# DeJhon-Huang/TrueTrace-Unity-Pathtracer

Measured on AMD Instinct MI355X. Metric: Mrays/sec (primary+1-bounce) on Sponza CWBVH at 1080p; % HBM roofline, higher is better.
Workload: dtype f32

## Files before the change

### truetrace-unity-pathtracer_amd/csrc/tt_trace.hip

```cpp
#include "tt_launch.h"
#include "tt_wide.h"

#ifndef TT_LEAF_REFILL_MIN
#define TT_LEAF_REFILL_MIN (TT_LEAF_POOL ? 16 : TT_REFILL_MIN)
#endif

namespace {
template <int INFO, int LEAF = 0>
__device__ __forceinline__ bool write_record(const TraceArgs& A, uint32_t ray_index, uint32_t pix, float col_w,
                                             const Best& best, const LaneRay& wr, int32_t inst_mesh = 0,
                                             int32_t inst_tri_offset = 0) {
    tt_ray_data* R = A.rays + ray_index;
    const int32_t best_mesh = LEAF ? (best.tri_id != -1 ? inst_mesh : 0) : best.mesh_id;
    auto tri_offset_of_best = [&]() -> int32_t {
        if (LEAF) return best.tri_id != -1 ? inst_tri_offset : A.mesh[0].TriOffset;
        return A.mesh[best.mesh_id].TriOffset;
    };
    if (INFO != 0) {
        if (pix < A.n_pixels) {
            uint4 o;
            bool write = false;
            if (INFO == 1) {
                const int32_t to = tri_offset_of_best();
                o = make_uint4((uint32_t)best_mesh, (uint32_t)(best.tri_id - to),
// ... 28 lines not shown
                        } else {
                            o.x = __float_as_uint(w.dx * best.t + w.ox);
                            o.y = __float_as_uint(w.dy * best.t + w.oy);
                            o.z = __float_as_uint(w.dz * best.t + w.oz);
                        }
                    }
                    o.w = miss ? 1u : 0u;
                }
            }
            if (write) reinterpret_cast<uint4*>(A.info)[pix] = o;
        }
    }
    const uint32_t uv = (uint32_t)(best.u * 65535.0f) | ((uint32_t)(best.v * 65535.0f) << 16);
    const uint4 hit = make_uint4((uint32_t)best_mesh, (uint32_t)best.tri_id, __float_as_uint(best.t), uv);
    reinterpret_cast<uint4*>(R)[2] = hit;
    if (A.hits_out) {
        const u32x4 v = {hit.x, hit.y, hit.z, hit.w};
        __builtin_amdgcn_raw_buffer_store_b128(v, buffer_rsrc(A.hits_out, 0x7fffffff), (ray_index - A.ray_offset) << 4,
                                               0, 0);
    }
    return best.t != A.far_plane;
}

__device__ __forceinline__ void keep_record(const TraceArgs& A, uint32_t ray_index) {
    if (A.hits_out) {
        const uint4 h = reinterpret_cast<const uint4*>(A.rays + ray_index)[2];
        const u32x4 v = {h.x, h.y, h.z, h.w};
        __builtin_amdgcn_raw_buffer_store_b128(v, buffer_rsrc(A.hits_out, 0x7fffffff), (ray_index - A.ray_offset) << 4,
                                               0, 0);
    }
}

static_assert(TT_CHUNK_BIG == 64, "the adaptive order maps one dequeue (TT_CHUNK_BIG rays) to one 64-ray chunk");
#ifndef TT_ORDER_MIN_REPS
#define TT_ORDER_MIN_REPS 32
#endif
__device__ __forceinline__ void record_chunk_cost(const TraceArgs& A, bool swizzle, uint32_t ray_index, int32_t reps) {
    if (reps < TT_ORDER_MIN_REPS) return;
    const uint32_t local = ray_index - A.ray_offset;
    uint32_t c = local >> 6;
    if (swizzle) {
        const uint32_t py = fastdiv(local, A.div_width), px = local - py * A.width;
        c = (py >> 3) * (A.width >> 3) + (px >> 3);
    }
    atomicMax(A.chunk_cost + c, (uint32_t)reps);
}
}


namespace {
__device__ __forceinline__ bool root_leaf_hit(const RootLeaf& R, const LaneRay& r, float max_distance) {
    const float adjx = __uint_as_float(rl_byte(R.e, 0) << 23) * r.ix;
    const float adjy = __uint_as_float(rl_byte(R.e, 1) << 23) * r.iy;
    const float adjz = __uint_as_float(rl_byte(R.e, 2) << 23) * r.iz;
    const float orgx = r.ix * (R.px - r.ox);
    const float orgy = r.iy * (R.py - r.oy);
    const float orgz = r.iz * (R.pz - r.oz);
    const bool nx = r.dx < 0.0f, ny = r.dy < 0.0f, nz = r.dz < 0.0f;
    const uint32_t x_min = rl_byte(nx ? R.qhi : R.qlo, 0), x_max = rl_byte(nx ? R.qlo : R.qhi, 0);
    const uint32_t y_min = rl_byte(ny ? R.qhi : R.qlo, 1), y_max = rl_byte(ny ? R.qlo : R.qhi, 1);
    const uint32_t z_min = rl_byte(nz ? R.qhi : R.qlo, 2), z_max = rl_byte(nz ? R.qlo : R.qhi, 2);
    const float tminx = fma_((float)x_min, adjx, orgx);
    const float tminy = fma_((float)y_min, adjy, orgy);
    const float tminz = fma_((float)z_min, adjz, orgz);
    const float tmaxx = fma_((float)x_max, adjx, orgx);
    const float tmaxy = fma_((float)y_max, adjy, orgy);
    const float tmaxz = fma_((float)z_max, adjz, orgz);
    const float tmin = fmaxf(fmaxf(tminx, tminy), fmaxf(tminz, 1e-8f));
    float tmaxz_c;
    asm("v_min_f32 %0, %1, %2" : "=v"(tmaxz_c) : "v"(tmaxz), "v"(max_distance));
    const float tmax = fminf(fminf(tmaxx, tmaxy), tmaxz_c);
    return tmin < tmax;
}
}


template <bool STATS, bool MATCHECK, int INFO, bool IND, bool ORD, int LEAF = 0>
__device__ __forceinline__ void trace_body(const TraceArgs& A) {
    static_assert(!LEAF || (!STATS && !MATCHECK && !ORD), "the leaf-TLAS form has no stats / material / order variants");
    constexpr bool POOL = LEAF != 0 && TT_LEAF_POOL != 0;
    constexpr bool ROOTSTEP = POOL && TT_LEAF_ROOT_STEP != 0;
    constexpr bool RESTART = ROOTSTEP && TT_LEAF_RESTART != 0;
    static_assert(!RESTART || LEAF == 1, "the restart parks no world ray: the record write reads it back");
    constexpr int tt_lds_depth = lds_depth_of<LEAF>();
    static_assert(!POOL || TT_CHUNK_BIG == TT_WAVE, "the prepared-ray pool holds one chunk, one slot per lane");
    __shared__ uint2 s_stack[tt_lds_depth][TT_BLOCK];
    __shared__ uint4 s_pool[POOL ? 3 : 1][TT_BLOCK];
    (void)s_pool;
    LeafEntry L{};
    if (LEAF) L = load_leaf_mesh<true>(A.leaf, A.root.base_tri + firstbithigh(A.root.bits));
    uint32_t root_cg_x = 0, root_tg_x = 0, root_imask = 0;
    if (ROOTSTEP) {
        const NodeWords n = load_node_uniform(A.nodes, A.n_nodes, (uint32_t)L.off.w);
        root_cg_x = n.n1.x + (uint32_t)L.off.y;
        root_tg_x = n.n1.y + (uint32_t)L.off.x;
        root_imask = n.n0.w >> 24;
    }
    const uint32_t tid = threadIdx.x;
    zero_next_control(A.ctl_next, tid);
    const uint32_t gtid = blockIdx.x * TT_BLOCK + tid;
    const uint32_t spill_stride = gridDim.x * TT_BLOCK;
    uint2* __restrict__ spill = A.spill;
    (void)gtid;
    (void)spill_stride;
    (void)spill;
    const uint32_t lane = tid & (TT_WAVE - 1);
#ifdef TT_DIAG_BLOCKS
    if (tid < TT_DB_N) tt_db[tid] = 0ull;
    __syncthreads();
#endif

    uint32_t pool_next = 0, pool_end = 0, more = 1;
    const uint32_t wave_id = blockIdx.x * (TT_BLOCK / TT_WAVE) + (tid >> 6);
    SegState S{blockIdx.x % TT_SEGS, 0u, 0u};
    const uint32_t n_rays = IND ? launch_ray_count(A) : A.n_rays;
    const uint32_t n_tiles = (n_rays + 63u) >> 6;
    const bool swizzle = IND ? (A.tile_swizzle && n_rays == A.n_pixels) : (A.tile_swizzle != 0u);
    const __amdgpu_buffer_rsrc_t nodes = buffer_rsrc(A.nodes, A.n_nodes * (uint32_t)TT_NODE_STRIDE);
    const __amdgpu_buffer_rsrc_t tris = buffer_rsrc(A.tris, A.n_tris * (uint32_t)sizeof(TriPos));

    constexpr uint32_t TT_IDLE = 0x80000000u;
    uint32_t ray_index = 0;
    uint32_t pix = 0;
    float col_w = 0.0f;
    bool pending = false;
    LaneRay ray{}, wray{};
    Best best{};
    uint2 cg = make_uint2(0u, 0u), tg = make_uint2(0u, TT_IDLE);
    uint32_t oct = 0;
    int32_t stack_size = 0, tlas_ss = -1;
    int32_t NodeOffset = 0, TriOffset = 0, MatOffset = 0, mesh_id = -1, Reps = 0;
    if (LEAF) {
        NodeOffset = L.off.y;
        TriOffset = L.off.x;
        MatOffset = L.off.z;
        mesh_id = L.mesh_id;
    }
    uint32_t c_nodes = 0, c_tris = 0, c_blas = 0, c_acc = 0, c_rays = 0, c_hits = 0, c_reps = 0, c_ovf = 0;
    uint32_t d_iter = 0, d_node_lanes = 0, d_node_iters = 0, d_tri_lanes = 0, d_tri_iters = 0, d_active_lanes = 0;
    uint32_t d_lead_same = 0, d_uniform = 0;
    auto world_ray = [&]() -> LaneRay { return wray; };
    auto ray_of = [&](uint32_t widx) -> uint32_t {
        uint32_t local = widx;
        if (swizzle) {
            const uint32_t tw = A.width >> 3;
            const uint32_t t = widx >> 6, l = widx & 63u;
            const uint32_t ty = fastdiv(t, A.div_tiles), tx = t - ty * tw;
            local = (ty * 8u + (l >> 3)) * A.width + tx * 8u + (l & 7u);
        }
        return A.ray_offset + local;
    };
    (void)ray_of;
    uint64_t parked = 0ull;
    (void)parked;
    auto ray_index_of = [&](uint32_t v) -> uint32_t {
        if constexpr (RESTART) return ray_of(v);
        return v;
    };

#if TT_ROOT_LEAF
    const bool rl_ok = A.root.ok != 0u;
#endif
    auto enter_blas = [&]() {
            TT_DB(8);
            const uint32_t mo = firstbithigh(tg.y);
            tg.y &= ~(1u << mo);
            const LeafEntry e = load_leaf_mesh<true>(A.leaf, tg.x + mo);
            mesh_id = e.mesh_id;
            NodeOffset = e.off.y;
            TriOffset = e.off.x;
            bool ok = true;
            if (tg.y != 0u) TT_PUSH(tg, ok);
            if (ok && (cg.y & 0xff000000u)) TT_PUSH(cg, ok);
            tg.y = 0u;
            if (ok) {
                tlas_ss = stack_size;
                MatOffset = e.off.z;
                enter_object_space(e, ray, oct, cg);
                if (STATS) c_blas++;
            } else {
                tg.y = TT_IDLE;
                if (STATS) c_ovf++;
                TT_REPORT_OVERFLOW(A);
                keep_record(A, ray_index);
            }
    };
    auto finish_ray = [&]() {
        const bool hit = write_record<INFO, LEAF>(A, ray_index_of(ray_index), pix, col_w, best, world_ray(), mesh_id,
                                                  TriOffset);
        if (STATS) c_hits += hit ? 1u : 0u;
        (void)hit;
        if (ORD) record_chunk_cost(A, swizzle, ray_index, Reps);
    };
    auto start_from = [&](const uint32_t widx, const uint4 p0, const uint4 p1, const uint4 p2) {
        TT_DL(19, true);
        ray_index = RESTART ? widx : ray_of(widx);
        ray.ox = __uint_as_float(p0.x);
        ray.oy = __uint_as_float(p0.y);
        ray.oz = __uint_as_float(p0.z);
        ray.dx = __uint_as_float(p0.w);
        ray.dy = __uint_as_float(p1.x);
        ray.dz = __uint_as_float(p1.y);
        ray.ix = __uint_as_float(p1.z);
        ray.iy = __uint_as_float(p1.w);
        ray.iz = __uint_as_float(p2.x);
        pix = p2.y;
        if (ROOTSTEP) {
            col_w = -1.0f;
            oct = p2.z & 0x7fffffffu;
            const uint32_t inner = p2.w & 0xff000000u;
            cg = make_uint2(root_cg_x, inner ? (inner | root_imask) : 0u);
            tg = make_uint2(root_tg_x, p2.w & 0x00ffffffu);
            Reps = (p2.z & 0x80000000u) ? 2 : 1;
        } else {
            col_w = __uint_as_float(p2.z);
            oct = p2.w & 0x7fffffffu;
            cg = make_uint2((p2.w & 0x80000000u) ? (uint32_t)L.off.w : 0u, p2.w & 0x80000000u);
        }
        if (LEAF == 2) {
            const uint4* rp = reinterpret_cast<const uint4*>(A.rays + ray_index);
            const uint4 r0 = rp[0], r1 = rp[1];
            wray.ox = __uint_as_float(r0.x);
            wray.oy = __uint_as_float(r0.y);
            wray.oz = __uint_as_float(r0.z);
            wray.dx = __uint_as_float(r1.x);
            wray.dy = __uint_as_float(r1.y);
            wray.dz = __uint_as_float(r1.z);
        }
        best.t = A.far_plane;
        best.u = 0.0f;
        best.v = 0.0f;
        best.mesh_id = 0;
        best.tri_id = -1;
        if (!ROOTSTEP) tg = make_uint2(0u, 0u);
        stack_size = 0;
        if (!ROOTSTEP) Reps = 1;
    };
    (void)start_from;
    constexpr uint32_t REFILL_MIN = LEAF ? TT_LEAF_REFILL_MIN : TT_REFILL_MIN;
    while (true) {
        TT_DB(0);
        const uint64_t idle = __ballot((int32_t)tg.y < 0);
        const uint32_t n_idle = (uint32_t)__builtin_popcount((uint32_t)idle) + (uint32_t)__builtin_popcount((uint32_t)(idle >> 32));
        const bool pool_dry = !more && pool_next >= pool_end;
#if TT_DRAIN_PRIO
        if (pool_dry) __builtin_amdgcn_s_setprio(TT_DRAIN_PRIO);
#endif
        const bool to_wide = TT_WIDE && pool_dry && n_idle < TT_WAVE && TT_WAVE - n_idle <= TT_WIDE_ENTER;
        const uint32_t refill_min = RESTART && pool_next >= pool_end ? (uint32_t)TT_LEAF_RESTART_MIN : REFILL_MIN;
        if ((n_idle == TT_WAVE && pool_dry) || (n_idle >= refill_min && !pool_dry) || to_wide) {
            if (pending) {
                TT_DB(1);
                finish_ray();
                pending = false;
            }
            if constexpr (RESTART) {
                if (parked != 0ull) {
                    TT_DB(34);
                    if ((parked >> lane) & 1ull) {
                        TT_DL(35, true);
                        const uint4 k0 = s_pool[0][tid];
                        const uint2 k1 = reinterpret_cast<const uint2*>(&s_pool[1][tid])[0];
                        Best kb;
                        kb.tri_id = (int32_t)k0.x;
                        kb.t = __uint_as_float(k0.y);
                        kb.u = __uint_as_float(k0.z);
                        kb.v = __uint_as_float(k0.w);
                        kb.mesh_id = 0;
                        write_record<INFO, LEAF>(A, ray_of(k1.x), k1.y, -1.0f, kb, LaneRay{}, mesh_id, TriOffset);
                    }
                    parked = 0ull;
                    __builtin_amdgcn_fence(__ATOMIC_ACQ_REL, "wavefront");
                    __builtin_amdgcn_wave_barrier();
                }
            }
        }
        if (n_idle == TT_WAVE && pool_dry) break;
#if TT_WIDE
        if (to_wide) {
            TT_DB(13);
            WideState st{{ray, world_ray(), cg, tg, oct, stack_size, tlas_ss, NodeOffset, TriOffset, MatOffset, Reps,
                          ray_index_of(ray_index), tid, gtid, (int32_t)tg.y >= 0},
                         best, mesh_id, pix, col_w};
            regroup<2, LEAF>(st, __ballot((int32_t)tg.y >= 0), lane);
            auto finish_wide = [&](const WideState& w) {
                const bool hit = write_record<INFO, LEAF>(A, w.ray_index, w.pix, w.col_w, w.best, w.wray, mesh_id, TriOffset);
                if (STATS) c_hits += hit ? 1u : 0u;
                if (ORD) record_chunk_cost(A, swizzle, w.ray_index, w.Reps);
            };
            auto exhaust_wide = [&](const WideState& w, bool overflow) {
                keep_record(A, w.ray_index);
                if (ORD && !overflow) record_chunk_cost(A, swizzle, w.ray_index, w.Reps);
            };
            wide_phase<STATS, MATCHECK, 2, LEAF>(A, st, s_stack, spill, spill_stride, nodes, tris, lane,
                                           Counters{c_nodes, c_tris, c_blas, c_acc, c_hits, c_reps, c_ovf},
                                           finish_wide, exhaust_wide);
            break;
        }
#endif
        if (n_idle >= refill_min && !pool_dry) {
            TT_DB(2);
#if TT_LONG_PRIO
            if (__ballot((int32_t)tg.y >= 0 && Reps >= TT_LONG_PRIO) != 0ull) __builtin_amdgcn_s_setprio(TT_LONG_PRIO_LEVEL);
            else __builtin_amdgcn_s_setprio(0);
#endif
            const uint32_t avail = pool_end - pool_next;
            uint32_t new_base = 0, new_count = 0;
            if (avail < n_idle && more) {
                new_count = sched_reserve(A.ctl, n_rays, n_tiles, lane, n_idle - avail, wave_id, S, new_base);
                more = new_count > 0 ? 1u : 0u;
                if (ORD && A.order && new_count > 0)
                    new_base = (__builtin_amdgcn_readfirstlane(A.order[new_base >> 6]) << 6) | (new_base & 63u);
            }
            const PoolTake pt = pool_take<TT_UNIFORM_POOL != 0>(idle, n_idle, new_base, new_count, pool_next, pool_end, more);
            const uint32_t widx = pt.widx;
            pool_next = pt.pool_next;
            pool_end = pt.pool_end;
            more = pt.more;
            if constexpr (POOL) {
                const uint32_t pcol = tid - lane;
                const bool take = (int32_t)tg.y < 0 && widx != 0xffffffffu;
                const bool take_left = take && lane_prefix(idle) < min(avail, n_idle);
                auto start_ray = [&](const uint4 p0, const uint4 p1, const uint4 p2) { start_from(widx, p0, p1, p2); };
                uint4 p0 = make_uint4(0u, 0u, 0u, 0u), p1 = p0, p2 = p0;
                if (take_left) {
                    const uint32_t slot = pcol + (widx & 63u);
                    p0 = s_pool[0][slot];
                    p1 = s_pool[1][slot];
                    p2 = s_pool[2][slot];
                    if (ROOTSTEP) start_ray(p0, p1, p2);
                }
                __builtin_amdgcn_fence(__ATOMIC_ACQ_REL, "wavefront");
                __builtin_amdgcn_wave_barrier();
                if (new_count > 0) {
                    TT_DB(4);
                    uint4 q0 = make_uint4(0u, 0u, 0u, 0u), q1 = q0, q2 = q0;
                    NodeWords rn{};
                    if (ROOTSTEP) rn = load_node_uniform(A.nodes, A.n_nodes, (uint32_t)L.off.w);
                    if (lane < new_count) {
                        const uint4* rp = reinterpret_cast<const uint4*>(A.rays + ray_of(new_base + lane));
                        const uint4 r0 = rp[0], r1 = rp[1];
                        float cw = 0.0f;
                        if (INFO == 2) cw = (r0.w < A.n_pixels) ? A.colors[r0.w].Data[3] : 0.0f;
                        LaneRay r;
                        r.ox = __uint_as_float(r0.x);
                        r.oy = __uint_as_float(r0.y);
                        r.oz = __uint_as_float(r0.z);
                        r.dx = __uint_as_float(r1.x);
                        r.dy = __uint_as_float(r1.y);
                        r.dz = __uint_as_float(r1.z);
                        r.ix = rcp_rn(r.dx);
                        r.iy = rcp_rn(r.dy);
                        r.iz = rcp_rn(r.dz);
                        uint32_t o = 0u;
                        uint2 g = make_uint2(0u, 0u);
                        const bool root_hit = root_leaf_hit(A.root, r, A.far_plane);
                        TT_DL(29, root_hit);
                        if (root_hit) enter_object_space(L, r, o, g);
                        q0 = make_uint4(__float_as_uint(r.ox), __float_as_uint(r.oy), __float_as_uint(r.oz),
                                        __float_as_uint(r.dx));
                        q1 = make_uint4(__float_as_uint(r.dy), __float_as_uint(r.dz), __float_as_uint(r.ix),
                                        __float_as_uint(r.iy));
                        q2 = make_uint4(__float_as_uint(r.iz), r0.w, __float_as_uint(cw), o | g.y);
                        if (ROOTSTEP) {
                            if (INFO == 2 && !(cw == -1.0f || (float)A.bounce == cw)) q2.y = 0xffffffffu;
                            q2.z = o | g.y;
                            q2.w = 0u;
                            s_pool[0][tid] = q0;
                            s_pool[1][tid] = q1;
                            s_pool[2][tid] = q2;
                            if (root_hit) {
                                TT_DB(28);
                                s_pool[2][tid].w = node_intersect(rn.n0, rn.n1, rn.n2, rn.n3, rn.n4, r, o, A.far_plane);
                            }
                        }
                    }
                    if (!ROOTSTEP) {
                        s_pool[0][tid] = q0;
                        s_pool[1][tid] = q1;
                        s_pool[2][tid] = q2;
                    }
                }
                __builtin_amdgcn_fence(__ATOMIC_ACQ_REL, "wavefront");
                __builtin_amdgcn_wave_barrier();
                if (take && !take_left) {
                    const uint32_t slot = pcol + (widx & 63u);
                    p0 = s_pool[0][slot];
                    p1 = s_pool[1][slot];
                    p2 = s_pool[2][slot];
                    if (ROOTSTEP) start_ray(p0, p1, p2);
                }
                if (!ROOTSTEP && take) start_ray(p0, p1, p2);
            }
            if (!POOL && (int32_t)tg.y < 0 && widx != 0xffffffffu) {
                TT_DB(4);
                TT_DL(19, true);
                uint32_t local = widx;
                if (swizzle) {
                    const uint32_t tw = A.width >> 3;
                    const uint32_t t = widx >> 6, l = widx & 63u;
                    const uint32_t ty = fastdiv(t, A.div_tiles), tx = t - ty * tw;
                    local = (ty * 8u + (l >> 3)) * A.width + tx * 8u + (l & 7u);
                }
                ray_index = A.ray_offset + local;
                const uint4* rp = reinterpret_cast<const uint4*>(A.rays + ray_index);
                const uint4 r0 = rp[0], r1 = rp[1];
                pix = r0.w;
                if (INFO == 2) col_w = (pix < A.n_pixels) ? A.colors[pix].Data[3] : 0.0f;
                ray.ox = __uint_as_float(r0.x);
                ray.oy = __uint_as_float(r0.y);
                ray.oz = __uint_as_float(r0.z);
                ray.dx = __uint_as_float(r1.x);
                ray.dy = __uint_as_float(r1.y);
                ray.dz = __uint_as_float(r1.z);
                ray.ix = rcp_rn(ray.dx);
                ray.iy = rcp_rn(ray.dy);
                ray.iz = rcp_rn(ray.dz);
                best.t = A.far_plane;
                best.u = 0.0f;
                best.v = 0.0f;
                best.mesh_id = 0;
                best.tri_id = -1;
                tg = make_uint2(0u, 0u);
                stack_size = 0;
                if (LEAF) {
                    if (LEAF == 2) wray = ray;
                    cg = make_uint2(0u, 0u);
                    Reps = 1;
                    if (root_leaf_hit(A.root, ray, best.t)) enter_object_space(L, ray, oct, cg);
                }
                if (!LEAF) {
                    wray = ray;
                    oct = octant_inv4(ray);
                    cg = make_uint2(A.tlas_base, 0x80000000u);
                    tlas_ss = -1;
                    NodeOffset = (int32_t)A.tlas_base;
                    TriOffset = 0;
                    MatOffset = 0;
                    mesh_id = -1;
                    Reps = 0;
                }
                if (STATS) c_rays++;
#if TT_ROOT_LEAF
                if (!LEAF && rl_ok) {
                    const RootLeaf& RL = A.root;
                    const bool hit = root_leaf_hit(RL, ray, best.t);
                    cg = make_uint2(RL.base_child, 0u);
                    tg = make_uint2(RL.base_tri, hit ? RL.bits : 0u);
                    Reps = 1;
                    if (STATS) c_nodes++;
                    if (hit) enter_blas();
                }
#endif
            }
        }

        TT_DL(30, (int32_t)tg.y < 0);
        if (STATS) {
            const uint64_t nm = __ballot(tg.y == 0u && Reps < TT_MAX_REPS && (cg.y & 0xff000000u));
            const uint64_t am = __ballot((int32_t)tg.y >= 0);
            if (lane == 0) {
                d_iter++;
                d_node_lanes += (uint32_t)__popcll(nm);
                d_node_iters += nm ? 1u : 0u;
                d_active_lanes += (uint32_t)__popcll(am);
            }
        }
        if (tg.y == 0u) {
            TT_DB(5);
            if (Reps >= TT_MAX_REPS) {
                tg.y = TT_IDLE;
                if (STATS) c_reps++;
                keep_record(A, ray_index_of(ray_index));
                if (ORD) record_chunk_cost(A, swizzle, ray_index, Reps);
            } else if (cg.y & 0xff000000u) {
                const uint32_t child = take_child(cg, oct);
                bool ok = true;
                if (cg.y & 0xff000000u) {
                    TT_DB(7);
                    TT_PUSH(cg, ok);
                }
                if (ok) {
                    TT_DB(6);
                    TT_DL(17, true);
                    if (STATS) {
                        const uint32_t lead = __builtin_amdgcn_readfirstlane(child);
                        const uint64_t same = __ballot(child == lead), all = __ballot(true);
                        d_lead_same += child == lead ? 1u : 0u;
                        d_uniform += (same == all && lane == (uint32_t)__builtin_ctzll(all)) ? 1u : 0u;
                    }
                    const NodeWords n = load_node<TT_NODE_CPOL>(nodes, child);
                    const uint32_t hitmask = node_intersect(n.n0, n.n1, n.n2, n.n3, n.n4, ray, oct, best.t);
                    cg = node_group(hitmask, n, NodeOffset);
                    tg = tri_group(hitmask, n, TriOffset);
                    Reps++;
                    if (STATS) c_nodes++;
                } else {
                    tg.y = TT_IDLE;
                    if (STATS) c_ovf++;
                    TT_REPORT_OVERFLOW(A);
                    keep_record(A, ray_index_of(ray_index));
                }
            } else {
                tg = cg;
                cg = make_uint2(0u, 0u);
            }
            if (!LEAF && (int32_t)tg.y > 0 && tlas_ss == -1) enter_blas();
        }

        if (STATS) {
            const uint64_t tm = __ballot((int32_t)tg.y > 0);
            if (lane == 0) {
                d_tri_lanes += (uint32_t)__popcll(tm);
                d_tri_iters += tm ? 1u : 0u;
            }
        }
        if ((int32_t)tg.y > 0) {
            TT_DB(9);
            TT_DL(18, true);
            const uint32_t ti = firstbithigh(tg.y);
            tg.y &= ~(1u << ti);
            const bool acc = intersect_triangle<MATCHECK>(tris, A.mat, A.bounce == 0, A.flags, (int32_t)(tg.x + ti),
                                                          mesh_id, MatOffset, ray, best);
            if (STATS) {
                c_tris++;
                c_acc += acc ? 1u : 0u;
            }
        }

        if constexpr (RESTART) {
            const bool used_up = tg.y == 0u && (cg.y & 0xff000000u) == 0u;
            const bool finishing = used_up && stack_size == 0;
            if (used_up) {
                TT_DB(10);
                TT_DL(31, finishing);
                if (stack_size != 0) {
                    TT_DB(11);
                    TT_POP(cg);
                }
            }
            const uint64_t fin = __ballot(finishing);
            if (fin != 0ull) {
                TT_DB(32);
                const uint32_t n_fin = (uint32_t)__builtin_popcount((uint32_t)fin) + (uint32_t)__builtin_popcount((uint32_t)(fin >> 32));
                const uint32_t n_take = min(n_fin, pool_end - pool_next);
                if (finishing) {
                    const uint32_t rank = lane_prefix(fin);
                    if (rank < n_take) {
                        TT_DL(33, true);
                        const uint32_t widx = pool_next + rank;
                        const uint32_t slot = (tid - lane) + (widx & 63u);
                        const uint4 p0 = s_pool[0][slot], p1 = s_pool[1][slot], p2 = s_pool[2][slot];
#ifdef TT_TEST_PARK_SWAP
                        s_pool[0][slot] = make_uint4((uint32_t)best.tri_id, __float_as_uint(best.t), __float_as_uint(best.v),
                                                     __float_as_uint(best.u));
#else
                        s_pool[0][slot] = make_uint4((uint32_t)best.tri_id, __float_as_uint(best.t), __float_as_uint(best.u),
                                                     __float_as_uint(best.v));
#endif
                        reinterpret_cast<uint2*>(&s_pool[1][slot])[0] = make_uint2(ray_index, pix);
                        start_from(widx, p0, p1, p2);
                    } else {
                        pending = true;
                        tg.y = TT_IDLE;
                    }
                }
                if (n_take != 0u) {
                    const uint64_t m = n_take >= 64u ? ~0ull : ((1ull << n_take) - 1ull);
                    parked |= m << (pool_next & 63u);
                    pool_next += n_take;
                }
            }
        } else if (tg.y == 0u && (cg.y & 0xff000000u) == 0u) {
            TT_DB(10);
            TT_DL(31, stack_size == 0);
            if (stack_size == 0) TT_DB(32);
            if (stack_size != 0) {
                TT_DB(11);
                if (!LEAF && stack_size == tlas_ss) {
                    TT_DB(12);
                    leave_blas(A.tlas_base, world_ray(), NodeOffset, TriOffset, tlas_ss, ray, oct);
                }
                TT_POP(cg);
            } else {
                pending = true;
                tg.y = TT_IDLE;
            }
        }
    }

#ifdef TT_DIAG_BLOCKS
    __syncthreads();
    if (tid < TT_DB_N && A.diag_times && tt_db[tid]) atomicAdd(A.diag_times + tid, tt_db[tid]);
#endif
    if (STATS) {
        const uint32_t v[8] = {wave_sum(c_rays), wave_sum(c_nodes), wave_sum(c_tris), wave_sum(c_blas),
                               wave_sum(c_hits), wave_sum(c_reps), wave_sum(c_ovf), wave_sum(c_acc)};
        if (lane == 0) {
#pragma unroll
            for (int k = 0; k < 8; k++)
                if (v[k]) atomicAdd(&A.ctl->stats[k], (unsigned long long)v[k]);
            const uint32_t d[6] = {d_iter, d_node_iters, d_node_lanes, d_tri_iters, d_tri_lanes, d_active_lanes};
#pragma unroll
            for (int k = 0; k < 6; k++) atomicAdd(&A.ctl->diag[k], (unsigned long long)d[k]);
        }
        const uint32_t ls = wave_sum(d_lead_same), un = wave_sum(d_uniform);
        if (lane == 0) {
            atomicAdd(&A.ctl->diag[6], (unsigned long long)ls);
            atomicAdd(&A.ctl->diag[7], (unsigned long long)un);
        }
    }
}

template <bool STATS, bool MATCHECK, int INFO>
__global__ TT_BOUNDS void tt_trace_kernel(TraceArgs A) {
    trace_body<STATS, MATCHECK, INFO, false, false>(A);
}
template <bool MATCHECK, int INFO>
__global__ TT_BOUNDS void tt_trace_kernel_indirect(TraceArgs A) {
    trace_body<false, MATCHECK, INFO, true, false>(A);
}
template <int INFO>
__global__ __launch_bounds__(TT_BLOCK) __attribute__((amdgpu_waves_per_eu(5))) void tt_trace_kernel_ord(TraceArgs A) {
    trace_body<false, false, INFO, false, true>(A);
}
template <int INFO>
__global__ TT_BOUNDS void tt_trace_kernel_ord_mat(TraceArgs A) {
    trace_body<false, true, INFO, false, true>(A);
}
#ifndef TT_LEAF_WAVES
#define TT_LEAF_WAVES(INFO) 6
#endif
#define TT_LEAF_BOUNDS __launch_bounds__(TT_BLOCK) __attribute__((amdgpu_waves_per_eu(TT_LEAF_WAVES(INFO))))
#ifndef TT_LEAF_WRAY_RESIDENT
#define TT_LEAF_WRAY_RESIDENT 1
#endif
#define TT_LEAF_FORM(INFO) \
    ((INFO) == 2 && TT_LEAF_WRAY_RESIDENT && !(TT_LEAF_POOL && TT_LEAF_ROOT_STEP && TT_LEAF_RESTART) ? 2 : 1)
template <bool IND, int INFO>
__global__ TT_LEAF_BOUNDS void tt_trace_leaf_kernel(TraceArgs A) {
    trace_body<false, false, INFO, IND, false, TT_LEAF_FORM(INFO)>(A);
}

template <bool S, bool M, int I>
static hipError_t launch_one(const TraceArgs& a, bool leaf, uint32_t grid, hipStream_t st) {
    if constexpr (!S && !M) {
        if (leaf) {
            if (a.n_rays_dev) hipLaunchKernelGGL((tt_trace_leaf_kernel<true, I>), dim3(grid), dim3(TT_BLOCK), 0, st, a);
            else hipLaunchKernelGGL((tt_trace_leaf_kernel<false, I>), dim3(grid), dim3(TT_BLOCK), 0, st, a);
            return hipGetLastError();
        }
    }
    if constexpr (!S) {
        if (a.n_rays_dev) {
// ... 67 lines not shown
```

### truetrace-unity-pathtracer_amd/csrc/tt_traverse.h

```cpp
#ifndef TT_TRAVERSE_H
#define TT_TRAVERSE_H
#include "tt_device.h"

#define TT_WAVE 64
#ifndef TT_BLOCK
#define TT_BLOCK 64
#endif
#ifndef TT_SEGS
#define TT_SEGS 8
#endif
#ifndef TT_CHUNK_BIG
#define TT_CHUNK_BIG 64
#endif
#ifndef TT_REFILL_MIN
#define TT_REFILL_MIN 20
#endif
#ifndef TT_PUSH_FAST
#define TT_PUSH_FAST 1
#endif
#ifndef TT_DRAIN_PRIO
#define TT_DRAIN_PRIO 2
#endif
#ifndef TT_LONG_PRIO
#define TT_LONG_PRIO 64
#endif
#ifndef TT_LONG_PRIO_LEVEL
#define TT_LONG_PRIO_LEVEL 2
#endif
#ifndef TT_UNIFORM_POOL
#define TT_UNIFORM_POOL 1
#endif
#ifndef TT_LDS_STACK
#define TT_LDS_STACK 12
#endif
#ifndef TT_LEAF_POOL
#define TT_LEAF_POOL 1
#endif
#ifndef TT_LEAF_LDS_STACK
#define TT_LEAF_LDS_STACK 6
#endif
#ifndef TT_LEAF_ROOT_STEP
#define TT_LEAF_ROOT_STEP 1
#endif
#ifndef TT_LEAF_RESTART
#define TT_LEAF_RESTART 1
#endif
#ifndef TT_LEAF_RESTART_MIN
#define TT_LEAF_RESTART_MIN 16
#endif
#ifndef TT_WAVES_PER_EU
#define TT_WAVES_PER_EU 0
#endif
#if TT_WAVES_PER_EU > 0
#define TT_BOUNDS __launch_bounds__(TT_BLOCK, TT_WAVES_PER_EU)
#else
#define TT_BOUNDS __launch_bounds__(TT_BLOCK)
#endif

#ifdef TT_DIAG_BLOCKS
#define TT_DB_N 40
__shared__ unsigned long long tt_db[TT_DB_N];
#define TT_DB(k)                                                                               \
    do {                                                                                       \
        const uint64_t m_ = __ballot(1);                                                       \
        if ((threadIdx.x & 63u) == (uint32_t)__builtin_ctzll(m_)) atomicAdd(&tt_db[k], 1ull); \
    } while (0)
#define TT_DL(k, pred)                                                                         \
    do {                                                                                       \
        const uint64_t p_ = __ballot(pred), m_ = __ballot(1);                                  \
        if ((threadIdx.x & 63u) == (uint32_t)__builtin_ctzll(m_))                              \
            atomicAdd(&tt_db[k], (unsigned long long)__popcll(p_));                            \
    } while (0)
#else
#define TT_DB(k) \
    do {         \
    } while (0)
#define TT_DL(k, pred) \
    do {               \
    } while (0)
#endif

namespace {

struct LaneRay {
    float ox, oy, oz, dx, dy, dz, ix, iy, iz;
};

__device__ __forceinline__ float fma_(float a, float b, float c) { return __builtin_fmaf(a, b, c); }
__device__ __forceinline__ uint32_t firstbithigh(uint32_t x) { return 31u - (uint32_t)__builtin_clz(x); }

__device__ __forceinline__ uint32_t octant_inv4(const LaneRay& r) {
    return (r.dx < 0.0f ? 0u : 0x04040404u) | (r.dy < 0.0f ? 0u : 0x02020202u) |
           (r.dz < 0.0f ? 0u : 0x01010101u);
}


typedef uint32_t u32x4 __attribute__((ext_vector_type(4)));
__device__ __forceinline__ __amdgpu_buffer_rsrc_t buffer_rsrc(const void* base, uint32_t bytes) {
    return __builtin_amdgcn_make_buffer_rsrc(const_cast<void*>(base), 0, (int)bytes, 0x00020000);
}
#ifndef TT_TRI_CPOL
#define TT_TRI_CPOL 0
#endif
#ifndef TT_NODE_CPOL
#define TT_NODE_CPOL 0
#endif
template <int CPOL = 0>
__device__ __forceinline__ uint4 buffer_load16(__amdgpu_buffer_rsrc_t r, uint32_t off) {
    const u32x4 v = __builtin_amdgcn_raw_buffer_load_b128(r, off, 0, CPOL);
    return make_uint4(v.x, v.y, v.z, v.w);
}
typedef uint32_t u32x2 __attribute__((ext_vector_type(2)));
template <int CPOL = 0>
__device__ __forceinline__ uint2 buffer_load8(__amdgpu_buffer_rsrc_t r, uint32_t off) {
    const u32x2 v = __builtin_amdgcn_raw_buffer_load_b64(r, off, 0, CPOL);
    return make_uint2(v.x, v.y);
}
template <int CPOL = 0>
__device__ __forceinline__ uint32_t buffer_load4(__amdgpu_buffer_rsrc_t r, uint32_t off) {
    return __builtin_amdgcn_raw_buffer_load_b32(r, off, 0, CPOL);
}
static_assert(TT_NODE_STRIDE == 80 || TT_NODE_STRIDE == 128, "node stride: 80 (the reference array) or 128");
__device__ __forceinline__ uint32_t node_offset(uint32_t i) {
    if (TT_NODE_STRIDE == 128) return i << 7;
    uint32_t r;
    asm("v_lshl_add_u32 %0, %1, 2, %1\n\tv_lshlrev_b32 %0, 4, %0" : "=&v"(r) : "v"(i));
    return r;
}
__device__ __forceinline__ uint32_t tri_offset(uint32_t i) {
    uint32_t r;
    asm("v_lshl_add_u32 %0, %1, 1, %1\n\tv_lshlrev_b32 %0, 4, %0" : "=&v"(r) : "v"(i));
// ... 275 lines not shown
    R.u = u;
    R.v = v;
    R.cand = TT_IN_TRIANGLE(u, v) && (t > 0.0f && t < best_t);
    R.accept = R.cand;
    if (MATCHECK && R.accept) {
        const uint32_t mi = (uint32_t)(mat_offset + (int32_t)d.c.y);
        const uint32_t w = mi < M.n_mat ? M.word[mi] : 0u;
        if ((w >> TT_MATWORD_CUTOUT) & 1u) {
            const CutoutMat cm = M.cut[mi];
            if (sample_linear(M, align_uv(base_uv(M, tri_id, u, v), cm)) < cm.cutoff) R.accept = false;
        }
        const bool glass = (w >> TT_MATWORD_GLASS) & 1u;
        if ((tflags & TT_TRACE_IGNORE_GLASS) && glass) R.accept = false;
        if ((tflags & TT_TRACE_IGNORE_BACKFACING) && bounce0 && !glass && R.accept &&
            backfacing(__uint_as_float(d.a.w), __uint_as_float(d.b.x), __uint_as_float(d.b.y), __uint_as_float(d.b.z),
                       __uint_as_float(d.b.w), __uint_as_float(d.c.x), r))
            R.accept = false;
        if (bounce0 && ((w >> TT_FLAG_INVISIBLE) & 1u)) R.accept = false;
    }
    return R;
}
template <bool MATCHECK>
__device__ __forceinline__ TriCand triangle_candidate(__amdgpu_buffer_rsrc_t tris, const MatView& M, bool bounce0,
                                                      uint32_t tflags, int32_t tri_id, int32_t mat_offset,
                                                      const LaneRay& r, float best_t) {
    return triangle_test<MATCHECK>(triangle_load<MATCHECK>(tris, tri_id), M, bounce0, tflags, tri_id, mat_offset, r,
                                   best_t);
}

template <bool MATCHECK>
__device__ __forceinline__ bool intersect_triangle(__amdgpu_buffer_rsrc_t tris, const MatView& M, bool bounce0, uint32_t tflags,
                                                   int32_t tri_id, int32_t mesh_id, int32_t mat_offset,
                                                   const LaneRay& r, Best& best) {
    const TriCand c = triangle_candidate<MATCHECK>(tris, M, bounce0, tflags, tri_id, mat_offset, r, best.t);
    if (c.accept) {
        best.t = c.t;
        best.u = c.u;
        best.v = c.v;
        best.mesh_id = mesh_id;
        best.tri_id = tri_id;
    }
    return c.cand;
}

__device__ __forceinline__ uint32_t seg_lo(uint32_t n_tiles, uint32_t seg) {
    return (uint32_t)(((uint64_t)n_tiles * seg / TT_SEGS) << 6);
}
struct SegState {
    uint32_t seg;
    uint32_t dead;
    uint32_t est;
};
__device__ __forceinline__ uint32_t sched_reserve(TraceControl* ctl, uint32_t n_rays, uint32_t n_tiles, uint32_t lane,
                                                  uint32_t need, uint32_t wave_id, SegState& S, uint32_t& base) {
    while (S.dead != (1u << TT_SEGS) - 1u) {
        const uint32_t lo = seg_lo(n_tiles, S.seg);
        const uint32_t hi = min(seg_lo(n_tiles, S.seg + 1), n_rays);
        const uint32_t len = hi > lo ? hi - lo : 0u;
        const uint32_t want = max(need, (uint32_t)TT_CHUNK_BIG);
        uint32_t off = 0;
        TT_DB(3);
        if (lane == 0) off = atomicAdd(&ctl->seg_ticket[S.seg * 32u], want);
        off = __builtin_amdgcn_readfirstlane(off);
        if (off < len) {
            S.est = off + want;
            base = lo + off;
            return min(want, len - off);
        }
        S.dead |= 1u << S.seg;
        const uint32_t start = (S.seg + 1u + wave_id % (TT_SEGS - 1u)) % TT_SEGS;
#pragma unroll
        for (uint32_t k = 0; k < TT_SEGS; k++) {
            const uint32_t c = (start + k) % TT_SEGS;
            if (!((S.dead >> c) & 1u)) {
                S.seg = c;
                break;
            }
        }
        S.est = 0;
    }
    return 0u;
}

__device__ __forceinline__ uint32_t lane_prefix(uint64_t mask) {
    return __builtin_amdgcn_mbcnt_hi((uint32_t)(mask >> 32), __builtin_amdgcn_mbcnt_lo((uint32_t)mask, 0u));
}

struct PoolTake {
    uint32_t widx, pool_next, pool_end, more;
};
template <bool UNIFORM>
__device__ __forceinline__ PoolTake pool_take(uint64_t idle, uint32_t n_idle, uint32_t new_base, uint32_t new_count,
                                              uint32_t pool_next, uint32_t pool_end, uint32_t more) {
    const uint32_t avail = pool_end - pool_next;
    const uint32_t take_old = min(avail, n_idle);
    const uint32_t take_new = min(n_idle - take_old, new_count);
    const uint32_t rank = lane_prefix(idle);
    uint32_t widx = 0xffffffffu;
    if (rank < take_old) widx = pool_next + rank;
    else if (rank - take_old < take_new) widx = new_base + (rank - take_old);
    if (new_count > 0) {
        pool_next = new_base + take_new;
        pool_end = new_base + new_count;
    } else {
        pool_next += take_old;
    }
    if (UNIFORM) {
        pool_next = __builtin_amdgcn_readfirstlane(pool_next);
        pool_end = __builtin_amdgcn_readfirstlane(pool_end);
        more = __builtin_amdgcn_readfirstlane(more);
    }
    return PoolTake{widx, pool_next, pool_end, more};
}

__device__ __forceinline__ void zero_next_control(TraceControl* next, uint32_t tid) {
    if (blockIdx.x == 0 && next) {
        uint32_t* w = reinterpret_cast<uint32_t*>(next);
        for (uint32_t i = tid; i < (uint32_t)(sizeof(TraceControl) / 4); i += TT_BLOCK) w[i] = 0u;
    }
}

__device__ __forceinline__ uint32_t wave_sum(uint32_t v) {
#pragma unroll
    for (int off = 32; off > 0; off >>= 1) v += __shfl_xor(v, off, TT_WAVE);
    return v;
}

template <class Kernel>
int occupancy_of(Kernel kernel) {
    int b = 0;
    return hipOccupancyMaxActiveBlocksPerMultiprocessor(&b, kernel, TT_BLOCK, 0) == hipSuccess ? b : 1;
}

}

namespace {
constexpr int tt_lds_depth = TT_LDS_STACK;
template <int LEAF>
constexpr int lds_depth_of() {
    return LEAF != 0 && TT_LEAF_POOL != 0 ? TT_LEAF_LDS_STACK : TT_LDS_STACK;
}
}
#if TT_PUSH_FAST
#define TT_PUSH(val, ok)                                                            \
    do {                                                                            \
        if (tt_lds_depth >= TT_STACK_SIZE || stack_size < tt_lds_depth) {           \
            if (tt_lds_depth >= TT_STACK_SIZE && stack_size == TT_STACK_SIZE) {     \
                ok = false;                                                         \
            } else {                                                                \
                s_stack[stack_size][tid] = (val);                                   \
                stack_size++;                                                       \
            }                                                                       \
        } else if (stack_size == TT_STACK_SIZE) {                                   \
            ok = false;                                                             \
        } else {                                                                    \
            spill[(size_t)(stack_size - tt_lds_depth) * spill_stride + gtid] = (val); \
            stack_size++;                                                           \
        }                                                                           \
    } while (0)
#else
#define TT_PUSH(val, ok)                                                            \
    do {                                                                            \
        if (stack_size == TT_STACK_SIZE) {                                          \
            ok = false;                                                             \
        } else {                                                                    \
            if (tt_lds_depth >= TT_STACK_SIZE || stack_size < tt_lds_depth)         \
// ... 18 lines not shown
```

Baseline: 7743.

## Add ready-state pool packing, raw ballots, deferred pop and uniform segment state

Adds several leaf-restart micro-optimisations, all on by default. The pooled ray slot now holds a pre-decoded traversal state (octant, inner mask, repetition count) so restarting a ray needs fewer decode ops. __ballot is replaced with the raw wave64 ballot builtin, and the stack pop is moved after the finish/restart step, so restarted rays no longer zero the stack. Empty node groups skip the tg/cg swap, and the scheduler segment state is forced wave-uniform. The combined changes risk subtle correctness issues, for example col_w is forced to -1 and the stack is not zeroed on restart.

```diff
diff --git a/truetrace-unity-pathtracer_amd/csrc/tt_trace.hip b/truetrace-unity-pathtracer_amd/csrc/tt_trace.hip
--- a/truetrace-unity-pathtracer_amd/csrc/tt_trace.hip
+++ b/truetrace-unity-pathtracer_amd/csrc/tt_trace.hip
@@ -134,6 +134,10 @@
     constexpr bool ROOTSTEP = POOL && TT_LEAF_ROOT_STEP != 0;
     constexpr bool RESTART = ROOTSTEP && TT_LEAF_RESTART != 0;
     static_assert(!RESTART || LEAF == 1, "the restart parks no world ray: the record write reads it back");
+    constexpr bool READY = RESTART && TT_LEAF_READY_STATE != 0;
+    constexpr bool MASKB = RESTART && TT_LEAF_MASK_BALLOT != 0;
+    constexpr bool POPLAST = RESTART && TT_LEAF_POP_LAST != 0;
+    constexpr bool EMPTYG = RESTART && TT_LEAF_EMPTY_GROUP != 0;
     constexpr int tt_lds_depth = lds_depth_of<LEAF>();
     static_assert(!POOL || TT_CHUNK_BIG == TT_WAVE, "the prepared-ray pool holds one chunk, one slot per lane");
     __shared__ uint2 s_stack[tt_lds_depth][TT_BLOCK];
@@ -238,13 +242,13 @@
             }
     };
     auto finish_ray = [&]() {
-        const bool hit = write_record<INFO, LEAF>(A, ray_index_of(ray_index), pix, col_w, best, world_ray(), mesh_id,
-                                                  TriOffset);
+        const bool hit = write_record<INFO, LEAF>(A, ray_index_of(ray_index), pix, READY ? -1.0f : col_w, best, world_ray(),
+                                                  mesh_id, TriOffset);
         if (STATS) c_hits += hit ? 1u : 0u;
         (void)hit;
         if (ORD) record_chunk_cost(A, swizzle, ray_index, Reps);
     };
-    auto start_from = [&](const uint32_t widx, const uint4 p0, const uint4 p1, const uint4 p2) {
+    auto start_from = [&](const uint32_t widx, const uint4 p0, const uint4 p1, const uint4 p2, const bool zero_stack) {
         TT_DL(19, true);
         ray_index = RESTART ? widx : ray_of(widx);
         ray.ox = __uint_as_float(p0.x);
@@ -257,7 +261,12 @@
         ray.iy = __uint_as_float(p1.w);
         ray.iz = __uint_as_float(p2.x);
         pix = p2.y;
-        if (ROOTSTEP) {
+        if (READY) {
+            oct = __builtin_amdgcn_perm(p2.z, p2.z, 0u);
+            cg = make_uint2(root_cg_x, __builtin_amdgcn_perm(p2.w, p2.z, 0x070c0c01u));
+            tg = make_uint2(root_tg_x, p2.w & 0x00ffffffu);
+            Reps = (int32_t)(p2.z >> 16);
+        } else if (ROOTSTEP) {
             col_w = -1.0f;
             oct = p2.z & 0x7fffffffu;
             const uint32_t inner = p2.w & 0xff000000u;
@@ -285,14 +294,14 @@
         best.mesh_id = 0;
         best.tri_id = -1;
         if (!ROOTSTEP) tg = make_uint2(0u, 0u);
-        stack_size = 0;
+        if (zero_stack) stack_size = 0;
         if (!ROOTSTEP) Reps = 1;
     };
     (void)start_from;
     constexpr uint32_t REFILL_MIN = LEAF ? TT_LEAF_REFILL_MIN : TT_REFILL_MIN;
     while (true) {
         TT_DB(0);
-        const uint64_t idle = __ballot((int32_t)tg.y < 0);
+        const uint64_t idle = lane_mask<MASKB>((int32_t)tg.y < 0);
         const uint32_t n_idle = (uint32_t)__builtin_popcount((uint32_t)idle) + (uint32_t)__builtin_popcount((uint32_t)(idle >> 32));
         const bool pool_dry = !more && pool_next >= pool_end;
 #if TT_DRAIN_PRIO
@@ -333,7 +342,7 @@
             TT_DB(13);
             WideState st{{ray, world_ray(), cg, tg, oct, stack_size, tlas_ss, NodeOffset, TriOffset, MatOffset, Reps,
                           ray_index_of(ray_index), tid, gtid, (int32_t)tg.y >= 0},
-                         best, mesh_id, pix, col_w};
+                         best, mesh_id, pix, READY ? -1.0f : col_w};
             regroup<2, LEAF>(st, __ballot((int32_t)tg.y >= 0), lane);
             auto finish_wide = [&](const WideState& w) {
                 const bool hit = write_record<INFO, LEAF>(A, w.ray_index, w.pix, w.col_w, w.best, w.wray, mesh_id, TriOffset);
@@ -353,7 +362,7 @@
         if (n_idle >= refill_min && !pool_dry) {
             TT_DB(2);
 #if TT_LONG_PRIO
-            if (__ballot((int32_t)tg.y >= 0 && Reps >= TT_LONG_PRIO) != 0ull) __builtin_amdgcn_s_setprio(TT_LONG_PRIO_LEVEL);
+            if (lane_mask<MASKB>((int32_t)tg.y >= 0 && Reps >= TT_LONG_PRIO) != 0ull) __builtin_amdgcn_s_setprio(TT_LONG_PRIO_LEVEL);
             else __builtin_amdgcn_s_setprio(0);
 #endif
             const uint32_t avail = pool_end - pool_next;
@@ -361,6 +370,10 @@
             if (avail < n_idle && more) {
                 new_count = sched_reserve(A.ctl, n_rays, n_tiles, lane, n_idle - avail, wave_id, S, new_base);
                 more = new_count > 0 ? 1u : 0u;
+                if constexpr (RESTART && TT_LEAF_UNIFORM_SEG != 0) {
+                    S.seg = __builtin_amdgcn_readfirstlane(S.seg);
+                    S.dead = __builtin_amdgcn_readfirstlane(S.dead);
+                }
                 if (ORD && A.order && new_count > 0)
                     new_base = (__builtin_amdgcn_readfirstlane(A.order[new_base >> 6]) << 6) | (new_base & 63u);
             }
@@ -373,7 +386,7 @@
                 const uint32_t pcol = tid - lane;
                 const bool take = (int32_t)tg.y < 0 && widx != 0xffffffffu;
                 const bool take_left = take && lane_prefix(idle) < min(avail, n_idle);
-                auto start_ray = [&](const uint4 p0, const uint4 p1, const uint4 p2) { start_from(widx, p0, p1, p2); };
+                auto start_ray = [&](const uint4 p0, const uint4 p1, const uint4 p2) { start_from(widx, p0, p1, p2, true); };
                 uint4 p0 = make_uint4(0u, 0u, 0u, 0u), p1 = p0, p2 = p0;
                 if (take_left) {
                     const uint32_t slot = pcol + (widx & 63u);
@@ -416,14 +429,20 @@
                         q2 = make_uint4(__float_as_uint(r.iz), r0.w, __float_as_uint(cw), o | g.y);
                         if (ROOTSTEP) {
                             if (INFO == 2 && !(cw == -1.0f || (float)A.bounce == cw)) q2.y = 0xffffffffu;
-                            q2.z = o | g.y;
+                            q2.z = READY ? ((o & 0xffu) | (root_hit ? 0x20000u : 0x10000u)) : (o | g.y);
                             q2.w = 0u;
                             s_pool[0][tid] = q0;
                             s_pool[1][tid] = q1;
                             s_pool[2][tid] = q2;
                             if (root_hit) {
                                 TT_DB(28);
-                                s_pool[2][tid].w = node_intersect(rn.n0, rn.n1, rn.n2, rn.n3, rn.n4, r, o, A.far_plane);
+                                const uint32_t hm = node_intersect(rn.n0, rn.n1, rn.n2, rn.n3, rn.n4, r, o, A.far_plane);
+                                if (READY) {
+                                    const uint32_t im = (hm & 0xff000000u) ? (rn.n0.w >> 24) << 8 : 0u;
+                                    reinterpret_cast<uint2*>(&s_pool[2][tid])[1] = make_uint2((o & 0xffu) | 0x20000u | im, hm);
+                                } else {
+                                    s_pool[2][tid].w = hm;
+                                }
                             }
                         }
                     }
@@ -553,7 +572,7 @@
                     TT_REPORT_OVERFLOW(A);
                     keep_record(A, ray_index_of(ray_index));
                 }
-            } else {
+            } else if (!EMPTYG) {
                 tg = cg;
                 cg = make_uint2(0u, 0u);
             }
@@ -583,15 +602,18 @@
         if constexpr (RESTART) {
             const bool used_up = tg.y == 0u && (cg.y & 0xff000000u) == 0u;
             const bool finishing = used_up && stack_size == 0;
+            const bool popping = used_up && stack_size != 0;
             if (used_up) {
                 TT_DB(10);
                 TT_DL(31, finishing);
-                if (stack_size != 0) {
+                if (!POPLAST && stack_size != 0) {
                     TT_DB(11);
                     TT_POP(cg);
                 }
             }
-            const uint64_t fin = __ballot(finishing);
+            const uint64_t fin = MASKB ? (lane_mask<MASKB>(tg.y == 0u) & lane_mask<MASKB>((cg.y & 0xff000000u) == 0u) &
+                                          lane_mask<MASKB>(stack_size == 0))
+                                       : lane_mask<false>(finishing);
             if (fin != 0ull) {
                 TT_DB(32);
                 const uint32_t n_fin = (uint32_t)__builtin_popcount((uint32_t)fin) + (uint32_t)__builtin_popcount((uint32_t)(fin >> 32));
@@ -604,14 +626,26 @@
                         const uint32_t slot = (tid - lane) + (widx & 63u);
                         const uint4 p0 = s_pool[0][slot], p1 = s_pool[1][slot], p2 = s_pool[2][slot];
 #ifdef TT_TEST_PARK_SWAP
-                        s_pool[0][slot] = make_uint4((uint32_t)best.tri_id, __float_as_uint(best.t), __float_as_uint(best.v),
-                                                     __float_as_uint(best.u));
+                        const float park_u = best.v, park_v = best.u;
 #else
-                        s_pool[0][slot] = make_uint4((uint32_t)best.tri_id, __float_as_uint(best.t), __float_as_uint(best.u),
-                                                     __float_as_uint(best.v));
-#endif
-                        reinterpret_cast<uint2*>(&s_pool[1][slot])[0] = make_uint2(ray_index, pix);
-                        start_from(widx, p0, p1, p2);
+                        const float park_u = best.u, park_v = best.v;
+#endif
+                        if (READY) {
+                            typedef __attribute__((address_space(3))) volatile uint32_t lds_word;
+                            lds_word* k0 = (lds_word*)&s_pool[0][slot];
+                            lds_word* k1 = (lds_word*)&s_pool[1][slot];
+                            k0[0] = (uint32_t)best.tri_id;
+                            k0[1] = __float_as_uint(best.t);
+                            k0[2] = __float_as_uint(park_u);
+                            k0[3] = __float_as_uint(park_v);
+                            k1[0] = ray_index;
+                            k1[1] = pix;
+                        } else {
+                            s_pool[0][slot] = make_uint4((uint32_t)best.tri_id, __float_as_uint(best.t), __float_as_uint(park_u),
+                                                         __float_as_uint(park_v));
+                            reinterpret_cast<uint2*>(&s_pool[1][slot])[0] = make_uint2(ray_index, pix);
+                        }
+                        start_from(widx, p0, p1, p2, !POPLAST);
                     } else {
                         pending = true;
                         tg.y = TT_IDLE;
@@ -622,6 +656,10 @@
                     parked |= m << (pool_next & 63u);
                     pool_next += n_take;
                 }
+            }
+            if (POPLAST && popping) {
+                TT_DB(11);
+                TT_POP(cg);
             }
         } else if (tg.y == 0u && (cg.y & 0xff000000u) == 0u) {
             TT_DB(10);
diff --git a/truetrace-unity-pathtracer_amd/csrc/tt_traverse.h b/truetrace-unity-pathtracer_amd/csrc/tt_traverse.h
--- a/truetrace-unity-pathtracer_amd/csrc/tt_traverse.h
+++ b/truetrace-unity-pathtracer_amd/csrc/tt_traverse.h
@@ -47,6 +47,21 @@
 #endif
 #ifndef TT_LEAF_RESTART_MIN
 #define TT_LEAF_RESTART_MIN 16
+#endif
+#ifndef TT_LEAF_READY_STATE
+#define TT_LEAF_READY_STATE 1
+#endif
+#ifndef TT_LEAF_MASK_BALLOT
+#define TT_LEAF_MASK_BALLOT 1
+#endif
+#ifndef TT_LEAF_POP_LAST
+#define TT_LEAF_POP_LAST 1
+#endif
+#ifndef TT_LEAF_EMPTY_GROUP
+#define TT_LEAF_EMPTY_GROUP 1
+#endif
+#ifndef TT_LEAF_UNIFORM_SEG
+#define TT_LEAF_UNIFORM_SEG 1
 #endif
 #ifndef TT_WAVES_PER_EU
 #define TT_WAVES_PER_EU 0
@@ -488,6 +503,12 @@
     return 0u;
 }
 
+template <bool MASK>
+__device__ __forceinline__ uint64_t lane_mask(bool p) {
+    if constexpr (MASK) return __builtin_amdgcn_ballot_w64(p);
+    return __ballot(p);
+}
+
 __device__ __forceinline__ uint32_t lane_prefix(uint64_t mask) {
     return __builtin_amdgcn_mbcnt_hi((uint32_t)(mask >> 32), __builtin_amdgcn_mbcnt_lo((uint32_t)mask, 0u));
 }
```

After: 7849 (median of 6 runs). 1.01x the previous value.
